# BKhomutenko/visgeom

Hardware: AMD Instinct MI355X
Metric: corner residual+Jacobian evals/sec (higher is better)
Workload: dtype f64; 1 GPU; EUCM mono, 10000 images x 96 corners (8x12 board) per GPU, chain [xiCamBoard DIRECT], residual + all Jacobian blocks (K=6 intrinsics + 6 pose) emitted to HBM in Ceres block layout; step = vg_problem_prepare + vg_dataset_evaluate (one launch: the emit kernel walks the single-member chain itself); images_per_gpu=10000, corners_per_image=96, camera_model=eucm, seed=20260929

## Files before the change

### visgeom_amd/csrc/vg_capi.hip

```cpp
#define VG_TU_CORE
#include <chrono>
#include <cstdio>
#include <cstdlib>
#include <cstring>
#include <new>
#include <string>
#include <vector>

#include "vg_internal.hpp"
#include "vg_gram.hpp"
#include "vg_gram_valu.hpp"
#include "vg_transf_host.hpp"

namespace {

thread_local std::string g_err;

}

int vgi::fail(int code, const std::string &msg)
{
    g_err = msg;
    return code;
}

using vgi::Camera;
using vgi::Dataset;
using vgi::Transform;
using vgi::fail;
using vgi::valid_dataset;

int vgi::check_device(int device, const char *what)
{
    int n = 0;
    const hipError_t e = hipGetDeviceCount(&n);
    if (e != hipSuccess || n <= 0) {
        (void)hipGetLastError();
        return fail(VG_ERR_NO_DEVICE, std::string("no HIP device available (") + (e == hipSuccess ? "device count 0" : hipGetErrorString(e)) +
                                          "): " + what + " has no CPU fallback");
    }
    if (device < 0 || device >= n) return fail(VG_ERR_INVALID_ARGUMENT, "device index out of range");
    return VG_OK;
}

namespace {

template <int MODEL>
size_t emit_lds_bytes(bool want_jac, bool frames_lds, int N, int frame_stride)
{
    size_t bytes = 0;
    bytes += (size_t)(vg::kEmitThreads / vg::kWave) * vg::emit_stage_doubles_per_wave<MODEL>() * sizeof(double);
    (void)want_jac;
    if (frames_lds) bytes += (size_t)(vg::kEmitThreads / N + 2) * frame_stride * sizeof(double);
    return bytes;
}

int64_t inline_chain_max_bytes()
{
    const long long h = vgi::debug_hook(vgi::kHookInlineChainMaxBytes);
    return h ? (int64_t)h : (int64_t)2000000000;
}

int64_t emit_nt_min_bytes()
{
    const long long h = vgi::debug_hook(vgi::kHookEmitNtMinBytes);
    return h ? (int64_t)h : (int64_t)230000000;
}

int emit_store_policy(int64_t launch_output_bytes)
{
    if (launch_output_bytes >= emit_nt_min_bytes()) return vg::kStoreNonTemporal;
    return vgi::debug_hook(vgi::kHookEmitWriteThrough) < 0 ? vg::kStorePlain : vg::kStoreWriteThrough;
}

unsigned int emit_map_window(int64_t launch_output_bytes)
{
    const long long mw = vgi::debug_hook(vgi::kHookEmitMapWindow);
    if (mw) return mw > 0 ? (unsigned int)mw : 0u;
    return launch_output_bytes >= (int64_t)1200000000 ? vg::kEmitMapWindow : 0u;
}

int64_t emit_output_bytes(const vg::EmitArgs &a, int K)
{
    int64_t per_obs = 16;
    if (a.jac_intr) per_obs += 16 * K;
    for (int l = 0; l < a.L; l++)
        if (a.jac_member[l]) per_obs += 96;
    return per_obs * (int64_t)a.n_obs;
}

bool emit_frames_in_lds(int N, int frame_stride)
{
    const int max_frames = vg::kEmitThreads / N + 2;
    return (size_t)max_frames * frame_stride * sizeof(double) <= 32 * 1024;
}

template <int MODEL, bool WANT_JAC, bool FRAMES_LDS, bool INLINE_CHAIN>
void launch_emit_policy(hipStream_t stream, const vg::EmitArgs &a, unsigned int grid, size_t lds)
{
    switch (a.nt_stores) {
    case vg::kStoreNonTemporal:
        hipLaunchKernelGGL((vg::vg_emit_kernel<MODEL, WANT_JAC, FRAMES_LDS, INLINE_CHAIN, vg::kStoreNonTemporal>), dim3(grid), dim3(vg::kEmitThreads), lds, stream, a);
        break;
    case vg::kStoreWriteThrough:
        hipLaunchKernelGGL((vg::vg_emit_kernel<MODEL, WANT_JAC, FRAMES_LDS, INLINE_CHAIN, vg::kStoreWriteThrough>), dim3(grid), dim3(vg::kEmitThreads), lds, stream, a);
        break;
    default:
        hipLaunchKernelGGL((vg::vg_emit_kernel<MODEL, WANT_JAC, FRAMES_LDS, INLINE_CHAIN, vg::kStorePlain>), dim3(grid), dim3(vg::kEmitThreads), lds, stream, a);
        break;
    }
}

template <int MODEL>
int launch_emit(hipStream_t stream, const vg::EmitArgs &a, bool want_jac, bool inline_chain)
{
    const bool frames_lds = emit_frames_in_lds((int)a.N, a.frame_stride_d);
    const size_t lds = emit_lds_bytes<MODEL>(want_jac, frames_lds, (int)a.N, a.frame_stride_d);
    const unsigned int grid = (a.n_obs + vg::kEmitThreads - 1) / vg::kEmitThreads;
    if (inline_chain) {
        if (want_jac) launch_emit_policy<MODEL, true, true, true>(stream, a, grid, lds);
        else launch_emit_policy<MODEL, false, true, true>(stream, a, grid, lds);
        VG_HIP(hipGetLastError());
        return VG_OK;
    }
    if (want_jac) {
        if (frames_lds)
            launch_emit_policy<MODEL, true, true, false>(stream, a, grid, lds);
        else
            launch_emit_policy<MODEL, true, false, false>(stream, a, grid, lds);
    } else {
        if (frames_lds)
            launch_emit_policy<MODEL, false, true, false>(stream, a, grid, lds);
        else
            launch_emit_policy<MODEL, false, false, false>(stream, a, grid, lds);
    }
    VG_HIP(hipGetLastError());
    return VG_OK;
}

bool dataset_can_inline_chain(const vg_problem *p, const Dataset &d)
{
    return d.L == 1 && d.status[0] == VG_TRANSFORM_DIRECT && emit_frames_in_lds(d.N, d.frame_stride) &&
           d.n_blocks * (int64_t)d.N * (32 + 16 * (p->cams[d.camera].K + 6)) <= inline_chain_max_bytes();
}

bool single_launch_dataset(const vg_problem *p, const Dataset &d)
{
    return !p->force_prepared_frames && dataset_can_inline_chain(p, d);
}

void fill_emit_args_at(const vg_problem *p, const Dataset &d, vg::EmitArgs &a, int64_t b0, int64_t nb, double *res_b0, double *ji_b0,
                       double *const *jm_b0)
{
    const Camera &cam = p->cams[d.camera];
    a.frames = d.d_frames + (size_t)b0 * d.frame_stride;
    a.board = d.d_board;
    a.obs = d.d_obs + (size_t)b0 * 2 * d.N;
    a.intr = p->d_params + cam.offset;
    a.res = res_b0;
    a.jac_intr = ji_b0;
    for (int l = 0; l < vg::kMaxChain; l++) a.jac_member[l] = (l < d.L && jm_b0) ? jm_b0[l] : nullptr;
    a.failed = d.d_failed;
    a.epoch = d.epoch;
    a.n_obs = (unsigned int)(nb * d.N);
    a.N = (unsigned int)d.N;
    a.L = d.L;
    a.frame_stride_d = d.frame_stride;
    a.chain_params = d.L ? p->d_params + d.chain.base[0] : nullptr;
    a.chain_stride = d.L ? d.chain.stride[0] : 0;
    a.seq_index = d.seq_identity ? nullptr : d.d_seq + b0;
    a.first_block = b0;
    a.nt_stores = emit_store_policy(emit_output_bytes(a, cam.K));
    a.map_window = emit_map_window(emit_output_bytes(a, cam.K));
}

void fill_emit_args(const vg_problem *p, const Dataset &d, vg::EmitArgs &a, int64_t b0, int64_t nb, double *residuals,
                    double *jac_intr, double *const *jac_member)
{
    const int K = p->cams[d.camera].K;
    double *jm[vg::kMaxChain] = {nullptr};
    for (int l = 0; l < d.L; l++)
        if (jac_member && jac_member[l]) jm[l] = jac_member[l] + (size_t)b0 * 2 * d.N * 6;
    fill_emit_args_at(p, d, a, b0, nb, residuals + (size_t)b0 * 2 * d.N, jac_intr ? jac_intr + (size_t)b0 * 2 * d.N * K : nullptr, jm);
}

}


#ifdef VG_DEBUG_HOOKS
namespace {
long long g_debug_hooks[vgi::kHookCount] = {0};
const char *const kDebugHookNames[vgi::kHookCount] = {"inline_chain_max_bytes", "gram_no_merge", "max_obs_per_launch", "solver_timing",
                                                      "solver_host_loop", "solver_device_loop", "solver_no_fold_frames", "solver_fold_max_groups",
                                                      "emit_nt_min_bytes", "host_chunk_bytes", "gram_persistent", "emit_map_window",
                                                      "emit_write_through"};
}
long long vgi::debug_hook(vgi::DebugHook h) { return g_debug_hooks[h]; }
#endif

extern "C" {

#ifdef VG_DEBUG_HOOKS
int vg_debug_set(const char *name, long long value)
{
    if (!name) return fail(VG_ERR_INVALID_ARGUMENT, "name is NULL");
    for (int k = 0; k < vgi::kHookCount; k++)
        if (std::strcmp(name, kDebugHookNames[k]) == 0) {
            g_debug_hooks[k] = value;
            return VG_OK;
        }
    return fail(VG_ERR_INVALID_ARGUMENT, std::string("unknown debug hook: ") + name);
}
#endif

int vg_abi_version(void) { return VG_ABI_VERSION; }

const char *vg_last_error(void) { return g_err.c_str(); }

int vg_device_count(void)
{
    int n = 0;
    if (hipGetDeviceCount(&n) != hipSuccess) return 0;
    return n;
}

int vg_num_intrinsics(int model) { return vg::num_intrinsics(model); }

int vg_intrinsic_bounds(int model, int idx, double *lower, double *upper)
{
    const int K = vg::num_intrinsics(model);
    if (K < 0 || idx < 0 || idx >= K || !lower || !upper) return fail(VG_ERR_INVALID_ARGUMENT, "bad model / index");
    double lo = 1., hi = 1e5;
    if (model == VG_MODEL_EUCM) {
        if (idx == 0) { lo = 0.; hi = 1.; }
        else if (idx == 1) { lo = 0.1; hi = 10.; }
    } else if (model == VG_MODEL_UCM) {
        if (idx == 0) { lo = 0.; hi = 3.; }
    } else {
        if (idx == 0) { lo = 0.; hi = 3.; }
        else if (idx <= 5) { lo = -10.; hi = 10.; }
    }
    *lower = lo;
    *upper = hi;
    return VG_OK;
}


int vg_problem_create(vg_problem **out, int device, void *hip_stream)
{
    if (!out) return fail(VG_ERR_INVALID_ARGUMENT, "out is NULL");
    *out = nullptr;
    int rc = vgi::check_device(device, "visgeom_amd");
    if (rc != VG_OK) return rc;
    VG_HIP(hipSetDevice(device));
    vg_problem *p = new (std::nothrow) vg_problem();
    if (!p) return fail(VG_ERR_ALLOC, "out of host memory");
    p->device = device;
    p->stream = reinterpret_cast<hipStream_t>(hip_stream);
    *out = p;
    return VG_OK;
}

void vg_problem_destroy(vg_problem *p)
{
    if (!p) return;
    (void)hipSetDevice(p->device);
    delete p;
}

int vg_problem_add_camera(vg_problem *p, int model, const double *intrinsics, int constant, int *camera_id)
{
    if (!p || !intrinsics) return fail(VG_ERR_INVALID_ARGUMENT, "NULL argument");
    if (p->finalized) return fail(VG_ERR_STATE, "problem already finalized");
    const int K = vg::num_intrinsics(model);
    if (K < 0) return fail(VG_ERR_INVALID_ARGUMENT, "unknown camera model");
    Camera c;
    c.model = model;
    c.K = K;
    c.constant = constant != 0;
    c.init.assign(intrinsics, intrinsics + K);
    p->cams.push_back(c);
    if (camera_id) *camera_id = (int)p->cams.size() - 1;
    return VG_OK;
}

int vg_problem_add_transform(vg_problem *p, int is_global, int constant, int count, const double *values,
                             int *transform_id)
{
    if (!p) return fail(VG_ERR_INVALID_ARGUMENT, "problem is NULL");
    if (p->finalized) return fail(VG_ERR_STATE, "problem already finalized");
    if (is_global) count = 1;
    if (count < 0) return fail(VG_ERR_INVALID_ARGUMENT, "negative transform count");
    Transform t;
    t.global = is_global != 0;
    t.constant = constant != 0;
    t.count = count;
    t.init.assign((size_t)count * 6, 0.);
    if (values) std::memcpy(t.init.data(), values, sizeof(double) * 6 * (size_t)count);
    p->tfs.push_back(t);
    if (transform_id) *transform_id = (int)p->tfs.size() - 1;
    return VG_OK;
}

}

namespace {
int add_dataset_common(vg_problem *p, int camera_id, int chain_len, const int *transform_ids, const int *status,
                       int n_points, const double *board, int64_t n_images, const int32_t *image_index,
                       const double *corners, const std::shared_ptr<vgi::CornerBlock> &resident, int *dataset_id)
{
    if (!p) return fail(VG_ERR_INVALID_ARGUMENT, "problem is NULL");
    if (p->finalized) return fail(VG_ERR_STATE, "problem already finalized");
    if (camera_id < 0 || camera_id >= (int)p->cams.size()) return fail(VG_ERR_INVALID_ARGUMENT, "camera id out of range");
    if (chain_len < 0 || chain_len > VG_MAX_CHAIN)
        return fail(VG_ERR_INVALID_ARGUMENT, "chain length must be in [0, 5]");
    if (chain_len > 0 && (!transform_ids || !status)) return fail(VG_ERR_INVALID_ARGUMENT, "chain arrays are NULL");
    if (n_points <= 0 || !board) return fail(VG_ERR_INVALID_ARGUMENT, "empty board");
    if (n_images < 0) return fail(VG_ERR_INVALID_ARGUMENT, "negative image count");
    Dataset d;
    d.camera = camera_id;
    d.L = chain_len;
    d.N = n_points;
    d.n_blocks = n_images;
    int64_t min_seq = -1;
    for (int l = 0; l < chain_len; l++) {
        const int t = transform_ids[l];
        if (t < 0 || t >= (int)p->tfs.size()) return fail(VG_ERR_INVALID_ARGUMENT, "transform id out of range");
        if (status[l] != VG_TRANSFORM_DIRECT && status[l] != VG_TRANSFORM_INVERSE)
            return fail(VG_ERR_INVALID_ARGUMENT, "status must be DIRECT or INVERSE");
        d.tids[l] = t;
        d.status[l] = status[l];
        if (!p->tfs[t].global && (min_seq < 0 || p->tfs[t].count < min_seq)) min_seq = p->tfs[t].count;
    }
    d.h_seq.resize((size_t)n_images);
    for (int64_t i = 0; i < n_images; i++) {
        const int64_t idx = image_index ? image_index[i] : i;
        if (idx < 0 || (min_seq >= 0 && idx >= min_seq))
            return fail(VG_ERR_INVALID_ARGUMENT, "image index outside the sequence transform");
        d.h_seq[(size_t)i] = (int32_t)idx;
    }
    d.h_board.assign(board, board + 3 * (size_t)n_points);
    if (resident) {
        if (resident->device != p->device || resident->N != n_points || resident->n_images < n_images)
            return fail(VG_ERR_INVALID_ARGUMENT, "the resident corner block does not fit the dataset (device, board size or image count)");
        d.resident = resident;
    } else {
        d.zero_obs = corners == nullptr;
        if (corners) d.h_obs.assign(corners, corners + (size_t)n_images * 2 * n_points);
// ... 268 lines not shown
int vgi::ensure_frames(vg_problem *p)
{
    if (!p->frames_stale) return VG_OK;
    const int rc = vgi::prepare_at(p, p->d_params);
    if (rc == VG_OK) p->frames_stale = false;
    return rc;
}

int vgi::prepare_at(vg_problem *p, const double *d_params)
{
    p->frames_stale = d_params != p->d_params;
    if (!p->prep_blocks) return VG_OK;
    if (p->d_prep) {
        const unsigned int grid = (unsigned int)((p->prep_blocks + 63) / 64);
        hipLaunchKernelGGL(vg::vg_chain_prep_table_kernel, dim3(grid), dim3(64), 0, p->stream, d_params, (const vg::PrepDataset *)p->d_prep,
                           (int)p->prep.size(), (long long)p->prep_blocks);
        VG_HIP(hipGetLastError());
        return VG_OK;
    }
    for (size_t g0 = 0; g0 < p->prep.size(); g0 += vg::kPrepMax) {
        vg::PrepMultiArgs m;
        m.n = (int)(p->prep.size() - g0 < (size_t)vg::kPrepMax ? p->prep.size() - g0 : (size_t)vg::kPrepMax);
        unsigned int waves = 0;
        int widest = 0;
        for (int k = 0; k < m.n; k++) {
            m.ds[k] = p->prep[g0 + (size_t)k];
            m.first_wave[k] = waves;
            waves += (unsigned int)((m.ds[k].count + 63) / 64);
            widest = m.ds[k].frame_stride_d > widest ? m.ds[k].frame_stride_d : widest;
        }
        for (int k = m.n; k <= vg::kPrepMax; k++) m.first_wave[k] = waves;
        m.staged = waves >= vg::kPrepStagedMinWaves ? 1 : 0;
        hipLaunchKernelGGL(vg::vg_chain_prep_multi_kernel, dim3(waves), dim3(64), m.staged ? (size_t)64 * widest * sizeof(double) : (size_t)0, p->stream, d_params, m);
        VG_HIP(hipGetLastError());
    }
    return VG_OK;
}

extern "C" {

int vg_problem_force_prepared_frames(vg_problem *p, int on)
{
    if (!p) return fail(VG_ERR_INVALID_ARGUMENT, "problem is NULL");
    p->force_prepared_frames = on != 0;
    p->frames_stale = true;
    return VG_OK;
}

int vg_problem_prepare(vg_problem *p)
{
    if (!p) return fail(VG_ERR_INVALID_ARGUMENT, "problem is NULL");
    if (!p->finalized) return fail(VG_ERR_STATE, "problem not finalized");
    VG_HIP(hipSetDevice(p->device));
    p->frames_stale = true;
    return VG_OK;
}

int vg_dataset_evaluate(vg_problem *p, int dataset_id, double *residuals, double *jac_intr, double *const *jac_member)
{
    int rc = valid_dataset(p, dataset_id);
    if (rc != VG_OK) return rc;
    if (!p->finalized) return fail(VG_ERR_STATE, "problem not finalized");
    Dataset &d = p->dss[dataset_id];
    d.epoch = (d.epoch + 1) & 0xFFFFFFull;
    if (d.epoch == 0) d.epoch = 1;
    if (!d.n_blocks) return VG_OK;
    if (!residuals) return fail(VG_ERR_INVALID_ARGUMENT, "residuals is NULL");
    VG_HIP(hipSetDevice(p->device));
    const Camera &cam = p->cams[d.camera];
    bool want_jac = jac_intr != nullptr;
    for (int l = 0; l < d.L; l++)
        if (jac_member && jac_member[l]) want_jac = true;
    const bool inline_chain = single_launch_dataset(p, d);
    if (!inline_chain && (rc = vgi::ensure_frames(p)) != VG_OK) return rc;

    int64_t max_obs = (int64_t)1 << 30;
    if (const long long h = vgi::debug_hook(vgi::kHookMaxObsPerLaunch)) max_obs = h > 0 ? h : max_obs;
    const int64_t max_blocks_per_launch = max_obs / d.N > 0 ? max_obs / d.N : 1;
    for (int64_t b0 = 0; b0 < d.n_blocks; b0 += max_blocks_per_launch) {
        const int64_t nb = d.n_blocks - b0 < max_blocks_per_launch ? d.n_blocks - b0 : max_blocks_per_launch;
        vg::EmitArgs a;
        fill_emit_args(p, d, a, b0, nb, residuals, jac_intr, jac_member);
        switch (cam.model) {
        case VG_MODEL_EUCM: rc = launch_emit<vg::kEUCM>(p->stream, a, want_jac, inline_chain); break;
        case VG_MODEL_UCM: rc = launch_emit<vg::kUCM>(p->stream, a, want_jac, inline_chain); break;
        default: rc = launch_emit<vg::kMEI>(p->stream, a, want_jac, inline_chain); break;
        }
        if (rc != VG_OK) return rc;
    }
    return VG_OK;
}

}

#include "vg_host_route.hpp"

extern "C" {

int vg_problem_evaluate(vg_problem *p, const vg_dataset_outputs *outs)
{
    if (!p || !outs) return fail(VG_ERR_INVALID_ARGUMENT, "NULL argument");
    if (!p->finalized) return fail(VG_ERR_STATE, "problem not finalized");
    VG_HIP(hipSetDevice(p->device));
    const int n_ds = (int)p->dss.size();
    int rc;
    std::vector<int> shared, alone;
    bool need_frames = false;
    for (int i = 0; i < n_ds; i++) {
        Dataset &d = p->dss[i];
        if (!d.n_blocks) {
            d.epoch = (d.epoch + 1) & 0xFFFFFFull;
            if (d.epoch == 0) d.epoch = 1;
            continue;
        }
        if (!outs[i].residuals) return fail(VG_ERR_INVALID_ARGUMENT, "residuals is NULL");
        bool want_jac = outs[i].jac_intr != nullptr;
        for (int l = 0; l < d.L; l++) want_jac = want_jac || outs[i].jac_member[l] != nullptr;
        if (want_jac && emit_frames_in_lds(d.N, d.frame_stride) && d.n_blocks * (int64_t)d.N < ((int64_t)1 << 30)) shared.push_back(i);
        else alone.push_back(i);
    }
    if (shared.size() < 2) {
        alone.insert(alone.end(), shared.begin(), shared.end());
        shared.clear();
    }
    std::stable_sort(shared.begin(), shared.end(), [&](int a2, int b2) {
        const Dataset &da = p->dss[a2], &db = p->dss[b2];
        return p->cams[da.camera].K + 6 * da.L > p->cams[db.camera].K + 6 * db.L;
    });
    for (int i : shared) need_frames = need_frames || !single_launch_dataset(p, p->dss[i]);
    if (need_frames && (rc = vgi::ensure_frames(p)) != VG_OK) return rc;
    for (size_t g0 = 0; g0 < shared.size(); g0 += vg::kEmitMultiMax) {
        vg::EmitMultiArgs m;
        m.n = (int)(shared.size() - g0 < (size_t)vg::kEmitMultiMax ? shared.size() - g0 : (size_t)vg::kEmitMultiMax);
        unsigned int tiles = 0;
        size_t lds = 0;
        for (int k = 0; k < m.n; k++) {
            Dataset &d = p->dss[shared[g0 + k]];
            const vg_dataset_outputs &o = outs[shared[g0 + k]];
            d.epoch = (d.epoch + 1) & 0xFFFFFFull;
            if (d.epoch == 0) d.epoch = 1;
            fill_emit_args(p, d, m.ds[k], 0, d.n_blocks, o.residuals, o.jac_intr, o.jac_member);
            m.model[k] = p->cams[d.camera].model;
            m.inline_chain[k] = single_launch_dataset(p, d) ? 1 : 0;
            m.first_tile[k] = tiles;
            tiles += (m.ds[k].n_obs + vg::kEmitThreads - 1) / vg::kEmitThreads;
            const size_t need = emit_lds_bytes<vg::kEUCM>(true, true, d.N, d.frame_stride);
            lds = need > lds ? need : lds;
        }
        for (int k = m.n; k <= vg::kEmitMultiMax; k++) m.first_tile[k] = tiles;
        {
            int64_t launch_bytes = 0;
            for (int k = 0; k < m.n; k++) launch_bytes += emit_output_bytes(m.ds[k], p->cams[p->dss[shared[g0 + k]].camera].K);
            for (int k = 0; k < m.n; k++) {
                m.ds[k].nt_stores = launch_bytes >= emit_nt_min_bytes() ? vg::kStoreNonTemporal : vg::kStorePlain;
                m.ds[k].map_window = emit_map_window(launch_bytes);
            }
        }
        unsigned int longest = 0;
        for (int k = 0; k < m.n; k++) longest += (m.first_tile[k + 1] - m.first_tile[k] + 7) / 8;
        if (m.ds[0].nt_stores == vg::kStoreNonTemporal)
            hipLaunchKernelGGL(vg::vg_emit_multi_kernel<vg::kStoreNonTemporal>, dim3(8 * longest), dim3(vg::kEmitThreads), lds, p->stream, m);
        else
            hipLaunchKernelGGL(vg::vg_emit_multi_kernel<vg::kStorePlain>, dim3(8 * longest), dim3(vg::kEmitThreads), lds, p->stream, m);
        VG_HIP(hipGetLastError());
    }
    for (int i : alone)
        if ((rc = vg_dataset_evaluate(p, i, outs[i].residuals, outs[i].jac_intr, outs[i].jac_member)) != VG_OK) return rc;
    return VG_OK;
}

int vg_problem_synchronize(vg_problem *p)
{
    if (!p) return fail(VG_ERR_INVALID_ARGUMENT, "problem is NULL");
    VG_HIP(hipSetDevice(p->device));
    VG_HIP(hipStreamSynchronize(p->stream));
    return VG_OK;
}

int vg_dataset_failed_count(vg_problem *p, int dataset_id, int64_t *count)
{
    int rc = valid_dataset(p, dataset_id);
    if (rc != VG_OK) return rc;
    if (!count) return fail(VG_ERR_INVALID_ARGUMENT, "count is NULL");
    if (!p->finalized) return fail(VG_ERR_STATE, "problem not finalized");
    VG_HIP(hipSetDevice(p->device));
    unsigned long long v = 0;
    VG_HIP(hipMemcpyAsync(&v, p->dss[dataset_id].d_failed, sizeof v, hipMemcpyDeviceToHost, p->stream));
    VG_HIP(hipStreamSynchronize(p->stream));
    const Dataset &d = p->dss[dataset_id];
    *count = (v >> 40) == d.epoch ? (int64_t)(v & ((1ull << 40) - 1)) : 0;
    return VG_OK;
}


int vg_dataset_gram_width(const vg_problem *p, int d)
{
    if (valid_dataset(p, d) != VG_OK) return -1;
    return p->cams[p->dss[d].camera].K + 6 * p->dss[d].L + 1;
}


}

extern "C" {



}

#include "vg_block_group.hpp"

namespace {

int block_new(vg_block **out, int device, int model, int chain_len, const int *status, int n_points, const double *grid,
              const double *obs)
{
    if (!out) return fail(VG_ERR_INVALID_ARGUMENT, "out is NULL");
    *out = nullptr;
    const int K = vg::num_intrinsics(model);
    if (K < 0) return fail(VG_ERR_INVALID_ARGUMENT, "unknown camera model");
    if (chain_len < 0 || chain_len > VG_MAX_CHAIN) return fail(VG_ERR_INVALID_ARGUMENT, "chain length must be in [0, 5]");
    if (chain_len > 0 && !status) return fail(VG_ERR_INVALID_ARGUMENT, "status is NULL");
    if (n_points <= 0 || !grid || !obs) return fail(VG_ERR_INVALID_ARGUMENT, "empty block");
    for (int l = 0; l < chain_len; l++)
        if (status[l] != VG_TRANSFORM_DIRECT && status[l] != VG_TRANSFORM_INVERSE)
            return fail(VG_ERR_INVALID_ARGUMENT, "status must be DIRECT or INVERSE");
    int rc = vgi::check_device(device, "visgeom_amd");
    if (rc != VG_OK) return rc;
    vg_block *b = new (std::nothrow) vg_block();
    if (!b) return fail(VG_ERR_ALLOC, "out of host memory");
    b->device = device;
    b->model = model;
    b->K = K;
    b->L = chain_len;
    b->N = n_points;
    for (int l = 0; l < chain_len; l++) b->status[l] = status[l];
    b->h_grid.assign(grid, grid + 3 * (size_t)n_points);
    b->h_obs.assign(obs, obs + 2 * (size_t)n_points);
    b->used.assign((size_t)K + 6 * (size_t)chain_len, 0.);
    *out = b;
    return VG_OK;
}

}

int vgg::ensure_private(vg_block *b)
{
    if (b->p) return VG_OK;
    int rc = vg_problem_create(&b->p, b->device, nullptr);
    std::vector<double> zeros(VG_MAX_INTRINSICS, 0.);
    int cam = -1, ds = -1, tids[vg::kMaxChain] = {0};
    if (rc == VG_OK) rc = vg_problem_add_camera(b->p, b->model, zeros.data(), 0, &cam);
    for (int l = 0; l < b->L && rc == VG_OK; l++) rc = vg_problem_add_transform(b->p, 1, 0, 1, nullptr, &tids[l]);
    if (rc == VG_OK) rc = vg_problem_add_dataset(b->p, cam, b->L, tids, b->status, b->N, b->h_grid.data(), 1, nullptr, b->h_obs.data(), &ds);
    if (rc == VG_OK) rc = vg_problem_finalize(b->p);
    if (rc == VG_OK) {
        const size_t rows = 2 * (size_t)b->N;
        const size_t total = rows * (1 + (size_t)b->K + 6 * (size_t)b->L);
        hipError_t e = b->d_out.alloc(sizeof(double) * total);
        if (e == hipSuccess) e = b->h_out.alloc(sizeof(double) * total, hipHostMallocDefault);
        if (e == hipSuccess) e = b->h_params.alloc(sizeof(double) * ((size_t)b->K + 6 * (size_t)b->L), hipHostMallocDefault);
        if (e != hipSuccess) rc = fail(VG_ERR_HIP, std::string("hipMalloc: ") + hipGetErrorString(e));
        else {
            b->d_res = b->d_out;
            b->d_jintr = b->d_out + rows;
            for (int l = 0; l < b->L; l++) b->d_jm[l] = b->d_out + rows * (1 + (size_t)b->K + 6 * (size_t)l);
        }
    }
    return rc;
}

namespace {

int block_evaluate_alone(vg_block *b, double const *const *parameters, double *residuals, double **jacobians)
{
    int rc = vgg::ensure_private(b);
    if (rc != VG_OK) return rc;
    std::memcpy(b->h_params, parameters[0], sizeof(double) * b->K);
    for (int l = 0; l < b->L; l++) std::memcpy(b->h_params + b->K + 6 * l, parameters[1 + l], sizeof(double) * 6);
    vg_problem *p = b->p;
    VG_HIP(hipSetDevice(p->device));
    hipStream_t s = p->stream;
    VG_HIP(hipMemcpyAsync(p->d_params, b->h_params, sizeof(double) * (size_t)p->n_params, hipMemcpyHostToDevice, s));
    p->frames_stale = true;
    double *jm[vg::kMaxChain] = {nullptr};
    double *ji = nullptr;
    size_t last = 2 * (size_t)b->N;
    const size_t rows = 2 * (size_t)b->N;
    if (jacobians) {
        if (jacobians[0]) {
            ji = b->d_jintr;
            last = rows * (1 + (size_t)b->K);
        }
        for (int l = 0; l < b->L; l++)
            if (jacobians[1 + l]) {
                jm[l] = b->d_jm[l];
                last = rows * (1 + (size_t)b->K + 6 * (size_t)(l + 1));
            }
    }
    rc = vg_dataset_evaluate(p, 0, b->d_res, ji, jm);
    if (rc != VG_OK) return rc;
    VG_HIP(hipMemcpyAsync(b->h_out, b->d_out, sizeof(double) * last, hipMemcpyDeviceToHost, s));
    VG_HIP(hipStreamSynchronize(s));
    std::memcpy(residuals, b->h_out, sizeof(double) * rows);
    if (ji) std::memcpy(jacobians[0], b->h_out + rows, sizeof(double) * rows * b->K);
    for (int l = 0; l < b->L; l++)
        if (jm[l]) std::memcpy(jacobians[1 + l], b->h_out + rows * (1 + (size_t)b->K + 6 * (size_t)l), sizeof(double) * rows * 6);
    return VG_OK;
}

void group_unseal(vg_block_group *g)
{
    if (g->p) vg_problem_destroy(g->p);
    g->p = nullptr;
// ... 230 lines not shown
```

### visgeom_amd/csrc/vg_internal.hpp

```cpp
#pragma once

#include "../../include/visgeom_amd.h"

#include <hip/hip_runtime.h>

#include <cstdint>
#include <functional>
#include <memory>
#include <string>
#include <vector>

#include "vg_kernels.hpp"
#include "vg_odometry.hpp"

namespace vgi {

int fail(int code, const std::string &msg);

enum DebugHook {
    kHookInlineChainMaxBytes = 0,
    kHookGramNoMerge,
    kHookMaxObsPerLaunch,
    kHookSolverTiming,
    kHookSolverHostLoop,
    kHookSolverDeviceLoop,
    kHookSolverNoFoldFrames,
    kHookSolverFoldMaxGroups,
    kHookEmitNtMinBytes,
    kHookHostChunkBytes,
    kHookGramPersistent,
    kHookEmitMapWindow,
    kHookEmitWriteThrough,
    kHookCount
};
#ifdef VG_DEBUG_HOOKS
long long debug_hook(DebugHook h);
#else
constexpr long long debug_hook(DebugHook) { return 0; }
#endif

#define VG_HIP(expr)                                                                              \
    do {                                                                                          \
        hipError_t e_ = (expr);                                                                   \
        if (e_ != hipSuccess) {                                                                   \
            return vgi::fail(e_ == hipErrorNoDevice || e_ == hipErrorInvalidDevice ? VG_ERR_NO_DEVICE \
                                                                                   : VG_ERR_HIP,  \
                             std::string(#expr) + ": " + hipGetErrorString(e_));                  \
        }                                                                                         \
    } while (0)

int check_device(int device, const char *what);

template <class H, hipError_t (*Free)(H)>
class HipOwner {
public:
    HipOwner() = default;
    HipOwner(HipOwner &&o) noexcept : h_(o.h_) { o.h_ = nullptr; }
    HipOwner &operator=(HipOwner &&o) noexcept
    {
        if (this != &o) {
            (void)release();
            h_ = o.h_;
            o.h_ = nullptr;
        }
        return *this;
    }
    ~HipOwner() { (void)release(); }
    hipError_t release()
    {
        H h = h_;
        h_ = nullptr;
        return h ? Free(h) : hipSuccess;
    }

protected:
    H h_ = nullptr;
};

template <class T>
struct DeviceMem : HipOwner<void *, hipFree> {
    T *get() const { return static_cast<T *>(h_); }
    operator T *() const { return get(); }
    hipError_t alloc(size_t bytes)
    {
        (void)release();
        return hipMalloc(&h_, bytes);
    }
};

template <class T>
struct PinnedMem : HipOwner<void *, hipHostFree> {
    T *get() const { return static_cast<T *>(h_); }
    operator T *() const { return get(); }
    hipError_t alloc(size_t bytes, unsigned int flags)
    {
        (void)release();
        return hipHostMalloc(&h_, bytes, flags);
    }
};

struct Stream : HipOwner<hipStream_t, hipStreamDestroy> {
    operator hipStream_t() const { return h_; }
    hipError_t create(unsigned int flags)
    {
        (void)release();
        return hipStreamCreateWithFlags(&h_, flags);
    }
};

struct Event : HipOwner<hipEvent_t, hipEventDestroy> {
    operator hipEvent_t() const { return h_; }
    hipError_t create(unsigned int flags = hipEventDefault)
    {
        (void)release();
        return hipEventCreateWithFlags(&h_, flags);
    }
};

struct StreamDrain {
    hipStream_t stream;
    bool armed = true;
    ~StreamDrain()
    {
        if (armed) (void)hipStreamSynchronize(stream);
    }
};

struct Camera {
    int model = 0, K = 0;
    bool constant = false;
    int64_t offset = -1;
    std::vector<double> init;
};

struct Transform {
    bool global = true, constant = false;
    int64_t count = 1;
    int64_t offset = -1;
    std::vector<double> init;
};

struct ParamBlock {
    int size = 0;
    bool constant = false;
    int64_t offset = -1;
    std::vector<double> init;
};

struct CornerBlock {
    int device = 0;
    DeviceMem<double> d_obs;
    int64_t n_images = 0;
    int N = 0;
};

struct Dataset {
    int camera = -1, L = 0, N = 0;
    int tids[vg::kMaxChain] = {0};
    int status[vg::kMaxChain] = {0};
    int64_t n_blocks = 0;
    std::vector<double> h_board, h_obs;
    std::vector<int32_t> h_seq;
    bool seq_identity = true;
    bool zero_obs = false;
    std::shared_ptr<CornerBlock> resident;
    double *d_obs = nullptr;
    DeviceMem<double> d_obs_own, d_board, d_frames;
    DeviceMem<int32_t> d_seq;
    DeviceMem<unsigned long long> d_failed;
    DeviceMem<double> d_host_stage;
    PinnedMem<double> h_host_stage;
    size_t d_host_stage_doubles = 0, h_host_stage_doubles = 0;
    Stream host_copy_stream;
    std::vector<Event> host_chunk_ready, host_chunk_copied;
    DeviceMem<double> d_partials;
    DeviceMem<double> d_wg_partials;
    unsigned long long epoch = 0;
    int frame_stride = 0;
    vg::ChainDesc chain;
};

struct Prior {
    int tf = -1;
    double A[36];
    double R[9];
// ... 83 lines not shown
```

### visgeom_amd/csrc/vg_kernels.hpp

```cpp
#pragma once

#include "vg_camera.hpp"

namespace vg {

constexpr int kMaxChain = 5;
constexpr int kEmitThreads = 256;
constexpr int kWave = 64;
constexpr double kDoubleBig = 1e15;

struct ChainDesc {
    int L;
    int status[kMaxChain];
    long long base[kMaxChain];
    long long stride[kMaxChain];
};

struct PrepDataset {
    ChainDesc chain;
    const int *seq_index;
    double *frames;
    long long first;
    long long count;
    int frame_stride_d;
};

constexpr int kPrepMax = 8;
struct PrepMultiArgs {
    PrepDataset ds[kPrepMax];
    unsigned int first_wave[kPrepMax + 1];
    int n;
    int staged;
};
constexpr unsigned int kPrepStagedMinWaves = 512;

#ifdef VG_TU_CORE
__global__ __launch_bounds__(64) void vg_chain_prep_table_kernel(const double *__restrict__ params,
                                                                  const PrepDataset *__restrict__ dsets, int n_dsets,
                                                                  long long total_blocks)
{
    const long long t = (long long)blockIdx.x * blockDim.x + threadIdx.x;
    if (t >= total_blocks) return;
    int d = 0;
    while (d + 1 < n_dsets && t >= dsets[d + 1].first) d++;
    const PrepDataset *D = dsets + d;
    const long long b = t - D->first;
    const int *seq = D->seq_index;
    const long long si = seq ? (long long)seq[b] : b;
    const long long *base = D->chain.base, *stride = D->chain.stride;
    build_frame(D->chain.L, D->chain.status, [&](int l) { return params + base[l] + stride[l] * si; },
                D->frames + b * D->frame_stride_d);
}

__global__ __launch_bounds__(64) void vg_chain_prep_multi_kernel(const double *__restrict__ params, PrepMultiArgs m)
{
    using d2 = HIP_vector_type<double, 2>;
    extern __shared__ __attribute__((aligned(16))) double prep_tile[];
    int d = 0;
    while (d + 1 < m.n && blockIdx.x >= m.first_wave[d + 1]) d++;
    const PrepDataset &D = m.ds[d];
    const long long b0 = (long long)(blockIdx.x - m.first_wave[d]) * 64;
    const long long b = b0 + threadIdx.x;
    const int stride = D.frame_stride_d, L = D.chain.L;
    if (b < D.count) {
        const int *seq = D.seq_index;
        const long long si = seq ? (long long)seq[b] : b;
        double xi[kMaxChain][6];
#pragma unroll
        for (int l = 0; l < kMaxChain; l++)
            if (l < L) {
                const double *src = params + D.chain.base[l] + D.chain.stride[l] * si;
#pragma unroll
                for (int k = 0; k < 6; k++) xi[l][k] = src[k];
            }
        auto walk = [&](double *frame) {
            ChainState s;
            chain_state_init(s);
#pragma unroll
            for (int l = 0; l < kMaxChain; l++)
                if (l < L) {
                    const Quat q1 = chain_acc_quat(s);
                    chain_walk_member(s, q1, xi[l], D.chain.status[l] != 0, frame + 12 + 21 * l);
                }
            chain_finish(s, frame);
        };
        if (!m.staged) {
            walk(D.frames + b * stride);
            return;
        }
        walk(prep_tile + threadIdx.x * stride);
    }
    if (!m.staged) return;
    __builtin_amdgcn_fence(__ATOMIC_RELEASE, "wavefront");
    __builtin_amdgcn_wave_barrier();
    __builtin_amdgcn_fence(__ATOMIC_ACQUIRE, "wavefront");
    const long long left = D.count - b0;
    const int total = (int)(left < 64 ? left : 64) * stride;
    double *dst = D.frames + b0 * stride;
    if ((reinterpret_cast<unsigned long long>(dst) & 15ull) == 0) {
        for (int i = threadIdx.x; i < (total >> 1); i += 64) reinterpret_cast<d2 *>(dst)[i] = reinterpret_cast<const d2 *>(prep_tile)[i];
        if ((total & 1) && threadIdx.x == 0) dst[total - 1] = prep_tile[total - 1];
    } else {
        for (int i = threadIdx.x; i < total; i += 64) dst[i] = prep_tile[i];
    }
}
#endif

struct EmitArgs {
    const double *frames;
    const double *board;
    const double *obs;
    const double *intr;
    double *res;
    double *jac_intr;
    double *jac_member[kMaxChain];
    unsigned long long *failed;
    unsigned long long epoch;
    const double *chain_params;
    const int *seq_index;
    long long chain_stride;
    long long first_block;
    unsigned int n_obs;
    unsigned int N;
    int L;
    int frame_stride_d;
    int nt_stores;
    unsigned int map_window;
};

enum EmitStorePolicy { kStorePlain = 0, kStoreNonTemporal = 1, kStoreWriteThrough = 2 };

template <int POLICY>
__device__ __forceinline__ void stream_store16(HIP_vector_type<double, 2> *dst, const HIP_vector_type<double, 2> &v)
{
    if constexpr (POLICY == kStoreNonTemporal) {
        __builtin_nontemporal_store(v.x, &dst->x);
        __builtin_nontemporal_store(v.y, &dst->y);
    } else if constexpr (POLICY == kStoreWriteThrough) {
        typedef unsigned int u4 __attribute__((ext_vector_type(4)));
        asm volatile("global_store_dwordx4 %0, %1, off sc1\n\ts_nop 1" ::"v"(dst), "v"(__builtin_bit_cast(u4, v)) : "memory");
    } else {
        *dst = v;
    }
}

template <int NK, int POLICY>
__device__ __forceinline__ void stream_tile_out(const HIP_vector_type<double, 2> *st, HIP_vector_type<double, 2> *dst, int n16, int lane)
{
    using d2 = HIP_vector_type<double, 2>;
    if constexpr (POLICY == kStoreNonTemporal) {
#pragma unroll
        for (int k = 0; k < NK; k++) {
            const int idx = k * kWave + lane;
            if (idx < n16) stream_store16<POLICY>(dst + idx, st[idx]);
        }
        return;
    }
    d2 v[NK];
#pragma unroll
    for (int k = 0; k < NK; k++) v[k] = st[k * kWave + lane];
    if (n16 >= NK * kWave) {
#pragma unroll
        for (int k = 0; k < NK; k++) stream_store16<POLICY>(dst + k * kWave + lane, v[k]);
    } else {
#pragma unroll
        for (int k = 0; k < NK; k++) {
            const int idx = k * kWave + lane;
            if (idx < n16) stream_store16<POLICY>(dst + idx, v[k]);
        }
    }
}

template <int S, int POLICY = kStorePlain>
__device__ __forceinline__ void wave_store_rows(double *__restrict__ stage, const double *vals,
                                                double *__restrict__ out_tile, int n_valid_obs, int lane)
{
    using d2 = HIP_vector_type<double, 2>;
    d2 *st = reinterpret_cast<d2 *>(stage);
#pragma unroll
    for (int i = 0; i < S; i++) {
        d2 v;
        v.x = vals[2 * i];
        v.y = vals[2 * i + 1];
        st[lane * S + i] = v;
    }
    __builtin_amdgcn_fence(__ATOMIC_RELEASE, "wavefront");
    __builtin_amdgcn_wave_barrier();
    __builtin_amdgcn_fence(__ATOMIC_ACQUIRE, "wavefront");
    stream_tile_out<S, POLICY>(st, reinterpret_cast<d2 *>(out_tile), n_valid_obs * S, lane);
    __builtin_amdgcn_fence(__ATOMIC_RELEASE, "wavefront");
    __builtin_amdgcn_wave_barrier();
    __builtin_amdgcn_fence(__ATOMIC_ACQUIRE, "wavefront");
}

constexpr int kStageRowDoubles = 6;

template <int MODEL>
constexpr int emit_stage_doubles_per_wave()
{
    return 2 * kWave * kStageRowDoubles;
}

template <int S, int POLICY>
__device__ __forceinline__ void wave_store_rows_halves(double *__restrict__ stage, const double *vals,
                                                       double *__restrict__ out_tile, int n_valid_obs, int lane)
{
    static_assert(S <= 2 * kStageRowDoubles, "half a wave of rows must fit the tile");
    using d2 = HIP_vector_type<double, 2>;
    d2 *st = reinterpret_cast<d2 *>(stage);
    constexpr int kHalf = kWave / 2;
#pragma unroll
    for (int h = 0; h < 2; h++) {
        if ((lane >> 5) == h) {
#pragma unroll
            for (int i = 0; i < S; i++) {
                d2 v;
                v.x = vals[2 * i];
                v.y = vals[2 * i + 1];
                st[(lane & (kHalf - 1)) * S + i] = v;
            }
        }
        __builtin_amdgcn_fence(__ATOMIC_RELEASE, "wavefront");
        __builtin_amdgcn_wave_barrier();
        __builtin_amdgcn_fence(__ATOMIC_ACQUIRE, "wavefront");
        int nv = n_valid_obs - h * kHalf;
        nv = nv < 0 ? 0 : (nv > kHalf ? kHalf : nv);
        stream_tile_out<(kHalf * S + kWave - 1) / kWave, POLICY>(st, reinterpret_cast<d2 *>(out_tile) + h * kHalf * S, nv * S, lane);
        __builtin_amdgcn_fence(__ATOMIC_RELEASE, "wavefront");
        __builtin_amdgcn_wave_barrier();
        __builtin_amdgcn_fence(__ATOMIC_ACQUIRE, "wavefront");
    }
}

__device__ __forceinline__ unsigned int xcd_contiguous_block(unsigned int b, unsigned int n)
{
    constexpr unsigned int kXcds = 8;
    const unsigned int x = b % kXcds, j = b / kXcds, q = n / kXcds, r = n % kXcds;
    return x * q + (x < r ? x : r) + j;
}

constexpr unsigned int kEmitMapWindow = 16;
__device__ __forceinline__ unsigned int xcd_window_block(unsigned int b, unsigned int n, unsigned int W)
{
    const unsigned int x = b & 7u, j = b >> 3, w = j / W, i = j - w * W, base = w * 8u * W, rem = n - base;
    if (rem >= 8u * W) return base + x * W + i;
    const unsigned int q = rem >> 3, r = rem & 7u;
    return base + x * q + (x < r ? x : r) + i;
}

template <int MODEL, bool WANT_JAC, int POLICY>
__device__ __forceinline__ void emit_tile_stores(const EmitArgs &a, const unsigned int o0, bool active, const HIP_vector_type<double, 2> &r,
                                                 const CornerEval<CameraTraits<MODEL>::K> &e, double X0, double X1, double X2,
                                                 const double *fr, double *stage)
{
    constexpr int K = CameraTraits<MODEL>::K;
    using d2 = HIP_vector_type<double, 2>;
    const int lane = threadIdx.x & (kWave - 1);
    if (active) stream_store16<POLICY>(reinterpret_cast<d2 *>(a.res) + o0 + threadIdx.x, r);

    if (WANT_JAC) {
        const unsigned int ow = o0 + (threadIdx.x & ~(kWave - 1));
        int n_valid = 0;
        if (ow < a.n_obs) n_valid = (a.n_obs - ow < (unsigned)kWave) ? (int)(a.n_obs - ow) : kWave;

        if (a.jac_intr) {
            double rows[2 * K];
#pragma unroll
            for (int i = 0; i < K; i++) {
                rows[i] = e.Ju[i];
                rows[K + i] = e.Jv[i];
            }
            if (K > kStageRowDoubles) wave_store_rows_halves<K, POLICY>(stage, rows, a.jac_intr + (size_t)ow * (2 * K), n_valid, lane);
            else wave_store_rows<(K > kStageRowDoubles ? 1 : K), POLICY>(stage, rows, a.jac_intr + (size_t)ow * (2 * K), n_valid, lane);
        }
        for (int l = 0; l < a.L; l++) {
            double *Jm = a.jac_member[l];
            if (!Jm) continue;
            double rows[12];
            pose_rows(e.P, X0, X1, X2, fr + 12 + 21 * l, rows);
            wave_store_rows<6, POLICY>(stage, rows, Jm + (size_t)ow * 12, n_valid, lane);
        }
    }
}

template <int MODEL, bool WANT_JAC, bool FRAMES_LDS, bool INLINE_CHAIN, int POLICY>
__device__ __forceinline__ void emit_tile(const EmitArgs &a, const unsigned int o0)
{
    static_assert(!INLINE_CHAIN || FRAMES_LDS, "the inline chain writes its frames to LDS");
    constexpr int K = CameraTraits<MODEL>::K;
    using d2 = HIP_vector_type<double, 2>;
    extern __shared__ __attribute__((aligned(16))) double smem[];

    const int tid = threadIdx.x;
    const int lane = tid & (kWave - 1);
    const int wave = tid >> 6;
    const unsigned int o = o0 + tid;
    const bool active = o < a.n_obs;
    const unsigned int oc = active ? o : a.n_obs - 1;
    const unsigned int b = oc / a.N;
    const unsigned int c = oc - b * a.N;

    const double g0 = a.board[3 * c], g1 = a.board[3 * c + 1], g2 = a.board[3 * c + 2];
    const d2 ob = reinterpret_cast<const d2 *>(a.obs)[oc];

    const double *fr;
    if (FRAMES_LDS) {
        double *fr_lds = smem + (kEmitThreads / kWave) * emit_stage_doubles_per_wave<MODEL>();
        const unsigned int b_first = o0 / a.N;
        const unsigned int o_last = (o0 + kEmitThreads - 1 < a.n_obs) ? o0 + kEmitThreads - 1 : a.n_obs - 1;
        const unsigned int nf = o_last / a.N - b_first + 1;
        if (INLINE_CHAIN) {
            if (const unsigned int f = tid; f < nf) {
                const long long bi = (long long)b_first + f;
                const long long si = a.seq_index ? (long long)a.seq_index[bi] : a.first_block + bi;
                {
                    double xi_r[6];
#pragma unroll
                    for (int k = 0; k < 6; k++) xi_r[k] = (a.chain_params + a.chain_stride * si)[k];
                    build_frame_single_direct_fast(xi_r, fr_lds + f * a.frame_stride_d);
                }
            }
        } else {
            const int n16 = (int)(nf * (unsigned)a.frame_stride_d) >> 1;
            const d2 *src = reinterpret_cast<const d2 *>(a.frames + (size_t)b_first * a.frame_stride_d);
            d2 *dst = reinterpret_cast<d2 *>(fr_lds);
            for (int i = tid; i < n16; i += kEmitThreads) dst[i] = src[i];
        }
        __syncthreads();
        fr = fr_lds + (b - b_first) * a.frame_stride_d;
    } else {
        fr = a.frames + (size_t)b * a.frame_stride_d;
    }

    const double X0 = (fr[0] * g0 + fr[1] * g1 + fr[2] * g2) + fr[9];
    const double X1 = (fr[3] * g0 + fr[4] * g1 + fr[5] * g2) + fr[10];
    const double X2 = (fr[6] * g0 + fr[7] * g1 + fr[8] * g2) + fr[11];

    CornerEval<K> e;
    eval_corner<MODEL, WANT_JAC, WANT_JAC>(a.intr, X0, X1, X2, e);

    d2 r;
    r.x = e.ok ? e.u - ob.x : kDoubleBig;
    r.y = e.ok ? e.v - ob.y : kDoubleBig;
    asm volatile("" ::"v"(r.x), "v"(r.y));

    if (a.failed) {
        const unsigned long long m = __ballot(active && !e.ok);
        if (m && lane == 0) {
            const unsigned long long n = (unsigned long long)__popcll(m);
            unsigned long long old = *a.failed, assumed;
            do {
                assumed = old;
                const unsigned long long cnt = (assumed >> 40) == a.epoch ? (assumed & ((1ull << 40) - 1)) + n : n;
                old = atomicCAS(a.failed, assumed, (a.epoch << 40) | cnt);
            } while (old != assumed);
        }
    }

    emit_tile_stores<MODEL, WANT_JAC, POLICY>(a, o0, active, r, e, X0, X1, X2, fr, smem + wave * emit_stage_doubles_per_wave<MODEL>());
}

template <int MODEL, bool WANT_JAC, bool FRAMES_LDS, bool INLINE_CHAIN, int POLICY>
#ifndef VG_EMIT_WAVES
#define VG_EMIT_WAVES 4
#endif
#ifndef VG_EMIT_MULTI_WAVES
#define VG_EMIT_MULTI_WAVES 4
#endif
__global__ __launch_bounds__(kEmitThreads) __attribute__((amdgpu_waves_per_eu(VG_EMIT_WAVES, 8))) void vg_emit_kernel(EmitArgs a)
{
    const unsigned int t = a.map_window ? xcd_window_block(blockIdx.x, gridDim.x, a.map_window) : xcd_contiguous_block(blockIdx.x, gridDim.x);
    emit_tile<MODEL, WANT_JAC, FRAMES_LDS, INLINE_CHAIN, POLICY>(a, t * (unsigned)kEmitThreads);
}

constexpr int kEmitMultiMax = 8;

struct EmitMultiArgs {
    EmitArgs ds[kEmitMultiMax];
    unsigned int first_tile[kEmitMultiMax + 1];
    int model[kEmitMultiMax];
    int inline_chain[kEmitMultiMax];
    int n;
};

template <int MODEL, int POLICY>
__device__ __forceinline__ void emit_tile_route(const EmitArgs &a, unsigned int o0, bool inline_chain)
{
    if (inline_chain) emit_tile<MODEL, true, true, true, POLICY>(a, o0);
    else emit_tile<MODEL, true, true, false, POLICY>(a, o0);
}

#ifdef VG_TU_CORE
template <int POLICY>
__global__ __launch_bounds__(kEmitThreads) __attribute__((amdgpu_waves_per_eu(VG_EMIT_MULTI_WAVES, 8))) void vg_emit_multi_kernel(EmitMultiArgs m)
{
    const unsigned int x = blockIdx.x & 7u;
    unsigned int j = blockIdx.x >> 3, t;
    int d = 0;
    for (;; d++) {
        if (d == m.n) return;
        const unsigned int nt = m.first_tile[d + 1] - m.first_tile[d], q = nt >> 3, r = nt & 7u, cnt = q + (x < r ? 1u : 0u);
        if (j < cnt) {
            const unsigned int W = m.ds[d].map_window;
            t = m.first_tile[d] + (W ? xcd_window_block(j * 8u + x, nt, W) : x * q + (x < r ? x : r) + j);
            break;
        }
        j -= cnt;
    }
    const unsigned int o0 = (t - m.first_tile[d]) * (unsigned)kEmitThreads;
    const bool inl = m.inline_chain[d] != 0;
    switch (m.model[d]) {
    case kEUCM: emit_tile_route<kEUCM, POLICY>(m.ds[d], o0, inl); break;
    case kUCM: emit_tile_route<kUCM, POLICY>(m.ds[d], o0, inl); break;
    default: emit_tile_route<kMEI, POLICY>(m.ds[d], o0, inl); break;
    }
}
#endif

constexpr int kStreamUnroll = 4;

#ifdef VG_TU_CORE
__global__ __launch_bounds__(256) void vg_stream_write_kernel(double *__restrict__ dst, long long n2, double value)
{
    using d2 = HIP_vector_type<double, 2>;
    d2 v;
    v.x = value;
    v.y = value;
    d2 *d = reinterpret_cast<d2 *>(dst);
    const long long base = (long long)blockIdx.x * (256 * kStreamUnroll) + threadIdx.x;
#pragma unroll
    for (int k = 0; k < kStreamUnroll; k++) {
        const long long i = base + k * 256;
        if (i < n2) d[i] = v;
    }
}
#endif

#ifdef VG_TU_CORE
__global__ __launch_bounds__(256) void vg_stream_copy_kernel(double *__restrict__ dst, const double *__restrict__ src,
                                                              long long n2)
{
    using d2 = HIP_vector_type<double, 2>;
    d2 *d = reinterpret_cast<d2 *>(dst);
    const d2 *s = reinterpret_cast<const d2 *>(src);
    const long long base = (long long)blockIdx.x * (256 * kStreamUnroll) + threadIdx.x;
    d2 t[kStreamUnroll];
#pragma unroll
    for (int k = 0; k < kStreamUnroll; k++) {
        const long long i = base + k * 256;
        if (i < n2) t[k] = s[i];
    }
#pragma unroll
    for (int k = 0; k < kStreamUnroll; k++) {
        const long long i = base + k * 256;
        if (i < n2) d[i] = t[k];
    }
}
#endif

constexpr int kFmaChains = 8;
#ifdef VG_TU_CORE
__global__ __launch_bounds__(256) void vg_fp64_fma_kernel(double *__restrict__ out, int iters, double seed)
{
    extern __shared__ double fma_pad[];
    double x[kFmaChains];
#pragma unroll
    for (int i = 0; i < kFmaChains; i++) x[i] = seed + 1e-3 * i + 1e-9 * threadIdx.x;
    const double a = 1.0000001, b = 1e-9;
#pragma unroll 4
    for (int k = 0; k < iters; k++)
#pragma unroll
        for (int i = 0; i < kFmaChains; i++) x[i] = __builtin_fma(x[i], a, b);
    double t = 0.;
#pragma unroll
    for (int i = 0; i < kFmaChains; i++) t += x[i];
    if (t == 12345.678) {
        fma_pad[threadIdx.x] = t;
        out[blockIdx.x] = fma_pad[threadIdx.x ^ 1];
    }
}
#endif

}
```

Measured before the change: 30.78 billion evals/s.

## Split emit tile into residual-first pass then Jacobian recompute, prefetch chain params

The single-dataset emit kernel now loads chain parameters at the very start of the tile, copies intrinsics into registers, and evaluates the corner without Jacobians first. It stores the residual right away, then re-evaluates with Jacobians and writes the Jacobian rows. The aim is to issue global loads and residual stores earlier so they overlap with the heavier Jacobian arithmetic. The cost is a second projection evaluation per corner and possibly more register pressure. It also adds optional timestamp instrumentation and routes the multi-dataset launch through the shared store-policy helper, which now includes a write-through variant.

```diff
diff --git a/visgeom_amd/csrc/vg_capi.hip b/visgeom_amd/csrc/vg_capi.hip
--- a/visgeom_amd/csrc/vg_capi.hip
+++ b/visgeom_amd/csrc/vg_capi.hip
@@ -172,6 +172,10 @@
     a.first_block = b0;
     a.nt_stores = emit_store_policy(emit_output_bytes(a, cam.K));
     a.map_window = emit_map_window(emit_output_bytes(a, cam.K));
+#ifdef VG_EMIT_STAMPS
+    a.stamps = reinterpret_cast<unsigned long long *>(vgi::debug_hook(vgi::kHookEmitStamps));
+    a.stamps_waves = (unsigned long long)vgi::debug_hook(vgi::kHookEmitStampsWaves);
+#endif
 }
 
 void fill_emit_args(const vg_problem *p, const Dataset &d, vg::EmitArgs &a, int64_t b0, int64_t nb, double *residuals,
@@ -193,7 +197,7 @@
 const char *const kDebugHookNames[vgi::kHookCount] = {"inline_chain_max_bytes", "gram_no_merge", "max_obs_per_launch", "solver_timing",
                                                       "solver_host_loop", "solver_device_loop", "solver_no_fold_frames", "solver_fold_max_groups",
                                                       "emit_nt_min_bytes", "host_chunk_bytes", "gram_persistent", "emit_map_window",
-                                                      "emit_write_through"};
+                                                      "emit_write_through", "emit_stamps", "emit_stamps_waves"};
 }
 long long vgi::debug_hook(vgi::DebugHook h) { return g_debug_hooks[h]; }
 #endif
@@ -768,7 +772,7 @@
             int64_t launch_bytes = 0;
             for (int k = 0; k < m.n; k++) launch_bytes += emit_output_bytes(m.ds[k], p->cams[p->dss[shared[g0 + k]].camera].K);
             for (int k = 0; k < m.n; k++) {
-                m.ds[k].nt_stores = launch_bytes >= emit_nt_min_bytes() ? vg::kStoreNonTemporal : vg::kStorePlain;
+                m.ds[k].nt_stores = emit_store_policy(launch_bytes);
                 m.ds[k].map_window = emit_map_window(launch_bytes);
             }
         }
@@ -776,6 +780,8 @@
         for (int k = 0; k < m.n; k++) longest += (m.first_tile[k + 1] - m.first_tile[k] + 7) / 8;
         if (m.ds[0].nt_stores == vg::kStoreNonTemporal)
             hipLaunchKernelGGL(vg::vg_emit_multi_kernel<vg::kStoreNonTemporal>, dim3(8 * longest), dim3(vg::kEmitThreads), lds, p->stream, m);
+        else if (m.ds[0].nt_stores == vg::kStoreWriteThrough)
+            hipLaunchKernelGGL(vg::vg_emit_multi_kernel<vg::kStoreWriteThrough>, dim3(8 * longest), dim3(vg::kEmitThreads), lds, p->stream, m);
         else
             hipLaunchKernelGGL(vg::vg_emit_multi_kernel<vg::kStorePlain>, dim3(8 * longest), dim3(vg::kEmitThreads), lds, p->stream, m);
         VG_HIP(hipGetLastError());
diff --git a/visgeom_amd/csrc/vg_internal.hpp b/visgeom_amd/csrc/vg_internal.hpp
--- a/visgeom_amd/csrc/vg_internal.hpp
+++ b/visgeom_amd/csrc/vg_internal.hpp
@@ -31,6 +31,8 @@
     kHookGramPersistent,
     kHookEmitMapWindow,
     kHookEmitWriteThrough,
+    kHookEmitStamps,
+    kHookEmitStampsWaves,
     kHookCount
 };
 #ifdef VG_DEBUG_HOOKS
diff --git a/visgeom_amd/csrc/vg_kernels.hpp b/visgeom_amd/csrc/vg_kernels.hpp
--- a/visgeom_amd/csrc/vg_kernels.hpp
+++ b/visgeom_amd/csrc/vg_kernels.hpp
@@ -126,7 +126,22 @@
     int frame_stride_d;
     int nt_stores;
     unsigned int map_window;
+#ifdef VG_EMIT_STAMPS
+    unsigned long long *stamps;
+    unsigned long long stamps_waves;
+#endif
 };
+
+#ifdef VG_EMIT_STAMPS
+__device__ __forceinline__ void emit_stamp(const EmitArgs &a, int k)
+{
+    const unsigned long long w = (unsigned long long)blockIdx.x * (kEmitThreads / kWave) + (threadIdx.x >> 6);
+    if (a.stamps && w < a.stamps_waves && (threadIdx.x & (kWave - 1)) == 0) a.stamps[w * 4 + k] = wall_clock64();
+}
+#define VG_EMIT_STAMP(a, k) emit_stamp(a, k)
+#else
+#define VG_EMIT_STAMP(a, k) ((void)0)
+#endif
 
 enum EmitStorePolicy { kStorePlain = 0, kStoreNonTemporal = 1, kStoreWriteThrough = 2 };
 
@@ -249,19 +264,16 @@
 }
 
 template <int MODEL, bool WANT_JAC, int POLICY>
-__device__ __forceinline__ void emit_tile_stores(const EmitArgs &a, const unsigned int o0, bool active, const HIP_vector_type<double, 2> &r,
+__device__ __forceinline__ void emit_tile_rows(const EmitArgs &a, const unsigned int o0, const unsigned int o_end,
                                                  const CornerEval<CameraTraits<MODEL>::K> &e, double X0, double X1, double X2,
                                                  const double *fr, double *stage)
 {
     constexpr int K = CameraTraits<MODEL>::K;
-    using d2 = HIP_vector_type<double, 2>;
     const int lane = threadIdx.x & (kWave - 1);
-    if (active) stream_store16<POLICY>(reinterpret_cast<d2 *>(a.res) + o0 + threadIdx.x, r);
-
     if (WANT_JAC) {
         const unsigned int ow = o0 + (threadIdx.x & ~(kWave - 1));
         int n_valid = 0;
-        if (ow < a.n_obs) n_valid = (a.n_obs - ow < (unsigned)kWave) ? (int)(a.n_obs - ow) : kWave;
+        if (ow < o_end) n_valid = (o_end - ow < (unsigned)kWave) ? (int)(o_end - ow) : kWave;
 
         if (a.jac_intr) {
             double rows[2 * K];
@@ -283,9 +295,10 @@
     }
 }
 
-template <int MODEL, bool WANT_JAC, bool FRAMES_LDS, bool INLINE_CHAIN, int POLICY>
+template <int MODEL, bool WANT_JAC, bool FRAMES_LDS, bool INLINE_CHAIN, int POLICY, bool HEAD_FIRST = false>
 __device__ __forceinline__ void emit_tile(const EmitArgs &a, const unsigned int o0)
 {
+    VG_EMIT_STAMP(a, 0);
     static_assert(!INLINE_CHAIN || FRAMES_LDS, "the inline chain writes its frames to LDS");
     constexpr int K = CameraTraits<MODEL>::K;
     using d2 = HIP_vector_type<double, 2>;
@@ -294,9 +307,24 @@
     const int tid = threadIdx.x;
     const int lane = tid & (kWave - 1);
     const int wave = tid >> 6;
+    const unsigned int o_end = o0 + kEmitThreads < a.n_obs ? o0 + kEmitThreads : a.n_obs;
+    const unsigned int b_first = o0 / a.N;
+
+    const unsigned int nf = (o_end - 1) / a.N - b_first + 1;
+    double xi_r[6];
+    auto load_chain_params = [&]() {
+        if ((unsigned)tid < nf) {
+            const long long bi = (long long)b_first + tid;
+            const long long si = a.seq_index ? (long long)a.seq_index[bi] : a.first_block + bi;
+#pragma unroll
+            for (int k = 0; k < 6; k++) xi_r[k] = (a.chain_params + a.chain_stride * si)[k];
+        }
+    };
+    if (INLINE_CHAIN && HEAD_FIRST) load_chain_params();
+
     const unsigned int o = o0 + tid;
-    const bool active = o < a.n_obs;
-    const unsigned int oc = active ? o : a.n_obs - 1;
+    const bool active = o < o_end;
+    const unsigned int oc = active ? o : o_end - 1;
     const unsigned int b = oc / a.N;
     const unsigned int c = oc - b * a.N;
 
@@ -306,17 +334,10 @@
     const double *fr;
     if (FRAMES_LDS) {
         double *fr_lds = smem + (kEmitThreads / kWave) * emit_stage_doubles_per_wave<MODEL>();
-        const unsigned int b_first = o0 / a.N;
-        const unsigned int o_last = (o0 + kEmitThreads - 1 < a.n_obs) ? o0 + kEmitThreads - 1 : a.n_obs - 1;
-        const unsigned int nf = o_last / a.N - b_first + 1;
         if (INLINE_CHAIN) {
+            if (!HEAD_FIRST) load_chain_params();
             if (const unsigned int f = tid; f < nf) {
-                const long long bi = (long long)b_first + f;
-                const long long si = a.seq_index ? (long long)a.seq_index[bi] : a.first_block + bi;
                 {
-                    double xi_r[6];
-#pragma unroll
-                    for (int k = 0; k < 6; k++) xi_r[k] = (a.chain_params + a.chain_stride * si)[k];
                     build_frame_single_direct_fast(xi_r, fr_lds + f * a.frame_stride_d);
                 }
             }
@@ -327,6 +348,7 @@
             for (int i = tid; i < n16; i += kEmitThreads) dst[i] = src[i];
         }
         __syncthreads();
+        VG_EMIT_STAMP(a, 1);
         fr = fr_lds + (b - b_first) * a.frame_stride_d;
     } else {
         fr = a.frames + (size_t)b * a.frame_stride_d;
@@ -336,8 +358,12 @@
     const double X1 = (fr[3] * g0 + fr[4] * g1 + fr[5] * g2) + fr[10];
     const double X2 = (fr[6] * g0 + fr[7] * g1 + fr[8] * g2) + fr[11];
 
+    double intr[K];
+#pragma unroll
+    for (int i = 0; i < K; i++) intr[i] = a.intr[i];
     CornerEval<K> e;
-    eval_corner<MODEL, WANT_JAC, WANT_JAC>(a.intr, X0, X1, X2, e);
+    if (HEAD_FIRST) eval_corner<MODEL, false, false>(intr, X0, X1, X2, e);
+    else eval_corner<MODEL, WANT_JAC, WANT_JAC>(intr, X0, X1, X2, e);
 
     d2 r;
     r.x = e.ok ? e.u - ob.x : kDoubleBig;
@@ -357,7 +383,14 @@
         }
     }
 
-    emit_tile_stores<MODEL, WANT_JAC, POLICY>(a, o0, active, r, e, X0, X1, X2, fr, smem + wave * emit_stage_doubles_per_wave<MODEL>());
+    VG_EMIT_STAMP(a, 2);
+    if (active) stream_store16<POLICY>(reinterpret_cast<d2 *>(a.res) + o, r);
+
+    if (WANT_JAC) {
+        if (HEAD_FIRST) eval_corner<MODEL, true, true>(intr, X0, X1, X2, e);
+        emit_tile_rows<MODEL, WANT_JAC, POLICY>(a, o0, o_end, e, X0, X1, X2, fr, smem + wave * emit_stage_doubles_per_wave<MODEL>());
+    }
+    VG_EMIT_STAMP(a, 3);
 }
 
 template <int MODEL, bool WANT_JAC, bool FRAMES_LDS, bool INLINE_CHAIN, int POLICY>
@@ -370,7 +403,7 @@
 __global__ __launch_bounds__(kEmitThreads) __attribute__((amdgpu_waves_per_eu(VG_EMIT_WAVES, 8))) void vg_emit_kernel(EmitArgs a)
 {
     const unsigned int t = a.map_window ? xcd_window_block(blockIdx.x, gridDim.x, a.map_window) : xcd_contiguous_block(blockIdx.x, gridDim.x);
-    emit_tile<MODEL, WANT_JAC, FRAMES_LDS, INLINE_CHAIN, POLICY>(a, t * (unsigned)kEmitThreads);
+    emit_tile<MODEL, WANT_JAC, FRAMES_LDS, INLINE_CHAIN, POLICY, true>(a, t * (unsigned)kEmitThreads);
 }
 
 constexpr int kEmitMultiMax = 8;
```

Result: faster. 31.54 billion evals/s (median of 6 runs) (+2.5%).
